# celo-org/celo-bls-snark-rs

Measured on AMD Instinct MI355X. Metric: BLS12-377 G1 MSM scalar-muls/sec, higher is better.
Workload: dtype u32 limbs (28-bit radix, 64-bit column accumulators); 1 GPU; BLS12-377 G1 Pippenger MSM, 2^20 random bases/scalars per GPU, inputs resident in HBM; bases_per_gpu=1048576, window_bits=16, windows=16, buckets=524288

## Files before the change

celo-bls-snark-rs_amd/csrc/host_ifma.cpp:

```cpp
#include <immintrin.h>
#include <cstdint>
#include <cstring>
#include "fp_consts.h"

namespace {

typedef unsigned __int128 u128;
constexpr uint64_t M52 = (uint64_t(1) << 52) - 1;

template <int NL> struct V { __m512i l[NL]; };

template <int N> static bool geq(const uint64_t* a, const uint64_t* b) {
  for (int i = N - 1; i >= 0; i--) if (a[i] != b[i]) return a[i] > b[i];
  return true;
}
template <int N> static void sub_in_place(uint64_t* a, const uint64_t* b) {
  u128 br = 0;
  for (int i = 0; i < N; i++) { u128 d = (u128)a[i] - b[i] - (uint64_t)br; a[i] = (uint64_t)d; br = (d >> 64) & 1; }
}
template <int N> static void dbl_mod(uint64_t* x, const uint64_t* p) {
  uint64_t c = 0;
  for (int i = 0; i < N; i++) { uint64_t n = (x[i] << 1) | c; c = x[i] >> 63; x[i] = n; }
  if (geq<N>(x, p)) sub_in_place<N>(x, p);
}
// ... 120 lines not shown
    return m;
  }

  static inline bool dbl(Vn& a) {
    const Vn U = add(a, a);
    if (maybe_zero(a) & 2u) return false;
    const Vn A1 = pick(U, a, IDX(1, 8 + 0));
    const Vn T1 = mul(A1, A1);
    const Vn XX2 = add(T1, T1), M3 = add(XX2, T1);
    const Vn A2 = pick(U, pick(a, M3, IDX(0, 8 + 1)), IDX(1, 8 + 0, 8 + 1));
    const Vn B2 = pick(T1, M3, IDX(0, 0, 8 + 1));
    const Vn T2 = mul(A2, B2);
    const Vn S2 = add(T2, T2);
    const Vn X3 = sub<1>(pick(T2, T2, IDX(2)), pick(S2, S2, IDX(1)));
    const Vn SmX = sub<2>(pick(T2, T2, IDX(1)), X3);
    const Vn A3 = pick(pick(M3, T2, IDX(1, 8 + 0)), T1, IDX(0, 1, 8 + 0, 1));
    const Vn B3 = pick(SmX, a, IDX(0, 8 + 1, 8 + 2, 8 + 3));
    const Vn T3 = mul(A3, B3);
    const Vn Y3 = sub<0>(T3, pick(T3, T3, IDX(1)));
    a = pick(pick(X3, Y3, IDX(0, 8 + 0)), T3, IDX(0, 1, 8 + 2, 8 + 3));
    return true;
  }
  static inline bool add_pt(Vn& a, const Vn& b, int bo) {
    const Vn A1 = pick(a, b, IDX(0, 8 + bo + 0, 1, 8 + bo + 1, 2, 3));
    const Vn B1 = pick(a, b, IDX(8 + bo + 2, 2, 8 + bo + 3, 3, 8 + bo + 2, 8 + bo + 3));
    const Vn T1 = mul(A1, B1);
    const Vn D = sub<0>(pick(T1, T1, IDX(1, 3)), pick(T1, T1, IDX(0, 2)));
    if (maybe_zero(D) & 1u) return false;
    const Vn T2 = mul(D, D);
    const Vn A3 = pick(D, T1, IDX(0, 8 + 0, 8 + 4));
    const Vn B3 = pick(T2, T2, IDX(0, 0, 0));
    const Vn T3 = mul(A3, B3);
    const Vn Q2 = add(T3, T3);
    const Vn s = add(T3, pick(Q2, Q2, IDX(1)));
    const Vn X3 = sub<2>(pick(T2, T2, IDX(1)), s);
    const Vn QmX = sub<3>(pick(T3, T3, IDX(1)), X3);
    const Vn A4 = pick(D, T1, IDX(1, 8 + 2, 8 + 5));
    const Vn B4 = pick(QmX, T3, IDX(0, 8 + 0, 8 + 0));
    const Vn T4 = mul(A4, B4);
    const Vn Y3 = sub<0>(T4, pick(T4, T4, IDX(1)));
    a = pick(pick(X3, Y3, IDX(0, 8 + 0)), pick(T3, T4, IDX(2, 8 + 2)), IDX(0, 1, 8 + 0, 8 + 1));
    return true;
  }

  static int horner(const uint64_t* pts, size_t stride, const int32_t* order, int steps, uint64_t* out, int* out_inf) {
    const Consts& c = C();
    const Vn cin = bcast(c.c_in), cout = bcast(c.c_out);
    Vn acc;
    for (int j = 0; j < NL; j++) acc.l[j] = _mm512_setzero_si512();
    bool inf = true;
    alignas(64) uint64_t lanes[NL][8];
    for (int k = 0; k < steps; k++) {
      const bool nodbl = order[k] >= 0 && (order[k] & 0x40000000);
      if (!inf && !nodbl && !dbl(acc)) return 1;
      if (order[k] < 0) continue;
      const uint64_t* q = pts + (size_t)(order[k] & 0x3FFFFFFF) * stride;
      uint64_t zz = 0;
      for (int i = 0; i < N; i++) zz |= q[2 * N + i];
      if (zz == 0) continue;
      for (int e = 0; e < 4; e++) {
        uint64_t l[NL];
        to52<N, NL>(q + e * N, l);
        for (int j = 0; j < NL; j++) lanes[j][e] = l[j];
      }
      Vn b;
      for (int j = 0; j < NL; j++) b.l[j] = _mm512_load_si512((const void*)lanes[j]);
      b = mul(b, cin);
      if (inf) { acc = b; inf = false; continue; }
      if (!add_pt(acc, b, 0)) return 1;
    }
    *out_inf = inf ? 1 : 0;
    if (inf) { memset(out, 0, 4 * N * 8); return 0; }
    Vn r = mul(acc, cout);
    for (int j = 0; j < NL; j++) _mm512_store_si512((void*)lanes[j], r.l[j]);
    for (int e = 0; e < 4; e++) {
      uint64_t l[NL], w[N];
      for (int j = 0; j < NL; j++) l[j] = lanes[j][e];
      from52<N, NL>(l, w);
      if (geq<N>(w, P::P64)) sub_in_place<N>(w, P::P64);
      memcpy(out + e * N, w, 8 * N);
    }
    return 0;
  }
};

}

extern "C" int celo_ifma_horner_377(const uint64_t* pts, size_t stride, const int32_t* order, int steps, uint64_t* out, int* inf) {
  return Ifma<celo::P377, 8>::horner(pts, stride, order, steps, out, inf);
}
extern "C" int celo_ifma_horner_761(const uint64_t* pts, size_t stride, const int32_t* order, int steps, uint64_t* out, int* inf) {
  return Ifma<celo::P761, 15>::horner(pts, stride, order, steps, out, inf);
}
```

celo-bls-snark-rs_amd/csrc/msm_engine.h:

```cpp
#pragma once

namespace celo {

extern "C" int celo_ifma_available();
extern "C" int celo_ifma_horner_377(const uint64_t* pts, size_t stride, const int32_t* order, int steps, uint64_t* out, int* inf);
extern "C" int celo_ifma_horner_761(const uint64_t* pts, size_t stride, const int32_t* order, int steps, uint64_t* out, int* inf);
typedef int (*ifma_horner_fn)(const uint64_t*, size_t, const int32_t*, int, uint64_t*, int*);
template <class F> struct IfmaHorner { static constexpr ifma_horner_fn fn = nullptr; };
template <> struct IfmaHorner<Fp<P377>> { static constexpr ifma_horner_fn fn = &celo_ifma_horner_377; };
template <> struct IfmaHorner<Fp<P761>> { static constexpr ifma_horner_fn fn = &celo_ifma_horner_761; };

struct MsmTimings {
  float convert = 0, sort = 0, accumulate = 0, reduce = 0, total = 0;
};

}
#include "msm_ba.h"
namespace celo {
template <> struct BaCfg<G_761> { static constexpr bool enabled = true; };

struct MsmTuning {
  bool narrow_windows, use_glv, use_gls, gls_force, lane_bitsum, host_threads, seg_occupancy, side_convert, side_convert_all, fx_compact;
  uint32_t seg_min, seg_min_shard, bitsum_lanes_max_shard;
  int seg_halves;
  uint32_t bitsum_lanes_max;
  int ba_levels, ba_occ; uint32_t ba_rounds;
  int batched_affine;
  uint32_t host_chunks;
  uint32_t host_head_split, host_tail_split;
  static const MsmTuning& get() {
    static const MsmTuning t = [] {
      MsmTuning v;
      v.use_glv = true;
      v.use_gls = true;
      v.host_chunks = getenv("CELO_HOST_CHUNKS") ? (uint32_t)atoi(getenv("CELO_HOST_CHUNKS")) : 0xFFFFFFFFu;
      v.host_head_split = 0xFFFFFFFFu;
      v.host_tail_split = 0xFFFFFFFFu;
      v.batched_affine = getenv("CELO_BA") ? atoi(getenv("CELO_BA")) : 0;
      v.narrow_windows = true;
      v.gls_force = false;
      v.lane_bitsum = true;
      v.fx_compact = true;
      v.host_threads = true;
      v.seg_halves = 0;
      v.seg_min = 32u;
      v.seg_min_shard = 16u;
      v.seg_occupancy = true;
      v.side_convert = false;
      v.side_convert_all = false;
      v.ba_levels = 3; v.ba_occ = 2; v.ba_rounds = 2u;
      v.bitsum_lanes_max_shard = 21 * 1024;
      v.bitsum_lanes_max = 21 * 1024;
      return v;
    }();
    return t;
  }
};

template <class G> class MsmEngine {
 public:
  typedef typename G::F F;
  typedef PointIO<F> IO;
  static constexpr int SW = G::SCALAR_WORDS;

  ~MsmEngine() { release(); }
  void release() {
    if (arena) { (void)hipFree(arena); arena = nullptr; arena_bytes = 0; }
    if (fxs) { (void)hipFree(fxs); fxs = nullptr; fxs_bytes = 0; }
    for (void* p : {(void*)d_in_bases, (void*)d_in_scalars, (void*)d_in_inf})
      if (p) (void)hipFree(p);
    d_in_bases = nullptr; d_in_scalars = nullptr; d_in_inf = nullptr; cap_in = 0;
    if (h_out) { (void)hipHostFree(h_out); h_out = nullptr; }
    if (d_side_out) { (void)hipFree(d_side_out); d_side_out = nullptr; side_out_bytes = 0; }
    if (d_fx_scalars) { (void)hipFree(d_fx_scalars); d_fx_scalars = nullptr; cap_fx = 0; }
    for (int i = 0; i < 6; i++) if (ev[i]) { (void)hipEventDestroy(ev[i]); ev[i] = nullptr; }
    for (int i = 0; i < 2; i++) if (ev_side[i]) { (void)hipEventDestroy(ev_side[i]); ev_side[i] = nullptr; }
    for (hipEvent_t e : ev_copy) if (e) (void)hipEventDestroy(e);
    ev_copy.clear();
  }
  static int window_bits(size_t n) {
    if (G::SCALAR_BITS > 256) {
      if (n < 512) return 9;
      return n < (size_t(1) << 19) ? 13 : 16;
    }
    if (n < (size_t(1) << 15)) return 11;
    return n < (size_t(1) << 19) ? 15 : 16;
  }
  int force_c = 0;
  hipStream_t own_stream() { return stream_.get(); }
  bool narrow_windows = MsmTuning::get().narrow_windows;
  bool narrow_top(int c) const { return narrow_windows && c == 16; }
  bool big_subgroup_points = false;
  bool ark_zero_identity = false;
// ... 264 lines not shown
      const uint32_t E32 = (uint32_t)fx->E();
      hipLaunchKernelGGL((k_fixed_place<G>), dim3((E32 + 1023) / 1024 < 4096 ? (E32 + 1023) / 1024 : 4096), dim3(1024), 0, stream, d_fx_v8, d_fx_dg, d_fx_cnt + 128, d_digits_all,
                         d_remap, E32, n, fx->NV);
    } else if (fx) hipLaunchKernelGGL((k_fixed_digits<SW, G::SCALAR_BITS>), dim3((fx->n + 255) / 256), dim3(256), 0, stream, d_scalars, fx->tinf, d_digits_all, fx->n, (uint32_t)n_,
                               fx->cf, fx->W, fx->NV, fx->M);
    else if (glv) { if (launch_digits<4, GlvExpand<G>::BITS>(c, (const uint32_t*)(A + o_sc2), nullptr, d_digits_all, n, stream)) return 3; }
    else if (launch_digits<SW, G::SCALAR_BITS>(c, d_scalars, d_inf, d_digits_all, n, stream)) return 3;
    HIP_TRY(hipMemsetAsync(d_counts, 0, o_zero_end - o_counts, stream), 1);
    sort_windows(0, (uint32_t)nw, stream);
    hipLaunchKernelGGL((k_size_hist<G>), dim3(slots / 256 < 512 ? (slots + 255) / 256 : 512), dim3(256), 0, stream, d_plen, d_bins, slots);
    hipLaunchKernelGGL((k_size_scan<G>), dim3(1), dim3(1024), 0, stream, d_bins, d_nwork);
    hipLaunchKernelGGL((k_size_scatter<G>), dim3((slots + 4095) / 4096), dim3(1024), 0, stream, d_plen, d_bins, d_order, slots);
    if (side) HIP_TRY(hipStreamWaitEvent(stream, ev_side[1], 0), 1);
    HIP_TRY(hipEventRecord(ev[2], stream), 1);
    if constexpr (BaCfg<G>::enabled) if (use_ba) {
      uint32_t* d_ba_pts = (uint32_t*)(A + o_ba_pts);
      const int levels = MsmTuning::get().ba_levels;
      if (ba_occ == 2)
        hipLaunchKernelGGL((k_ba_levels<G, 2>), dim3(ba_lanes / 256), dim3(256), 0, stream, d_bases, d_sorted, d_pstart, d_plen, d_order, d_nwork, d_ba_pts,
                           (uint32_t*)(A + o_ba_pref), ba_lanes, levels, ba_pref_slots);
      else
        hipLaunchKernelGGL((k_ba_levels<G, 1>), dim3(ba_lanes / 256), dim3(256), 0, stream, d_bases, d_sorted, d_pstart, d_plen, d_order, d_nwork, d_ba_pts,
                           (uint32_t*)(A + o_ba_pref), ba_lanes, levels, ba_pref_slots);
      hipLaunchKernelGGL((k_accumulate_ba<G>), dim3((slots + 255) / 256), dim3(256), 0, stream, d_ba_pts, d_pstart, d_plen, d_order, d_nwork, d_partials, levels);
    }
    if (!use_ba) launch_accumulate<G>(slots, stream, d_bases, d_sorted, d_pstart, d_plen, d_order, d_nwork, d_partials);
    }
    HIP_TRY(hipEventRecord(ev[3], stream), 1);
    const uint32_t mid_blocks = win_cnt ? (total + 20) / 21 < 16384 ? (total + 20) / 21 : 16384 : 1024;
    const uint32_t cfirst = hin ? 1u : 0u;
    if (lane_bitsum) hipLaunchKernelGGL((k_combine_mid_lanes<G>), dim3(mid_blocks), dim3(64), 0, stream, d_mid, d_nmid, d_counts, d_pfirst, d_partials, d_piecesof, SEG, cfirst);
    else hipLaunchKernelGGL((k_combine_mid<G>), dim3(256), dim3(128), 0, stream, d_mid, d_nmid, d_counts, d_pfirst, d_partials, d_piecesof, SEG, cfirst);
    hipLaunchKernelGGL((k_combine_big<G>), dim3(256), dim3(256), 0, stream, d_big, d_nbig, d_counts, d_pfirst, d_partials, d_piecesof, SEG, cfirst);
    const uint32_t* d_leaf = d_partials;
    const uint32_t* d_leaf_counts = d_counts;
    if (hin) {
      hipLaunchKernelGGL((k_merge_carried<G>), dim3((total + 127) / 128), dim3(128), 0, stream, d_counts, d_pfirst, d_partials, d_carrier, total, K, SEG);
      d_leaf = d_carrier; d_leaf_counts = nullptr;
    }
    {
      struct Arr { uint32_t at, per_window; bool born; int level; };
      uint32_t half_at[2] = {res_pts, res_pts + half_pts};
      Arr tree = {0, B, true, LB};
      std::vector<Arr> lists;
      for (int t = 1; t <= LB; t++) {
        BitsumJobs jobs;
        jobs.njobs = 0;
        uint32_t cursor = half_at[t & 1], total_out = 0;
        auto push = [&](uint32_t src, uint32_t outs_per_window, uint32_t mode, int result_slot) -> uint32_t {
          const uint32_t outs = outs_per_window * (uint32_t)nw;
          uint32_t dst;
          if (result_slot >= 0) dst = (uint32_t)result_slot * (uint32_t)nw;
          else { dst = cursor; cursor += outs; }
          const int j = (int)jobs.njobs++;
          total_out += outs;
          jobs.end[j] = total_out; jobs.src[j] = src; jobs.dst[j] = dst; jobs.mode[j] = mode;
          return dst;
        };
        std::vector<Arr> next_lists;
        if (tree.level >= 2) {
          const uint32_t outs = tree.per_window / 4;
          const uint32_t dst = push(tree.at, outs, tree.level == LB ? 3u : 1u, outs == 1 ? tree.level : -1);
          if (outs > 1) next_lists.push_back({dst, outs, false, tree.level});
        } else {
          push(tree.at, 1, 4u, 1);
        }
        for (const Arr& L : lists) {
          const uint32_t outs = L.per_window / 2;
          const uint32_t dst = push(L.at, outs, 0u, outs == 1 ? L.level : -1);
          if (outs > 1) next_lists.push_back({dst, outs, false, L.level});
        }
        {
          const uint32_t outs = tree.per_window / 2;
          const uint32_t dst = push(tree.at, outs, tree.level == LB ? 2u : 0u, outs == 1 ? 0 : -1);
          tree = {dst, outs, true, tree.level - 1};
        }
        lists.swap(next_lists);
        if (lane_bitsum && total_out <= (win_cnt ? MsmTuning::get().bitsum_lanes_max_shard : BITSUM_LANES_MAX))
          hipLaunchKernelGGL((k_bitsum_lanes<G>), dim3((total_out + 20) / 21), dim3(64), 0, stream, d_leaf, d_leaf_counts, d_pfirst, d_piecesof, SEG, d_work, jobs);
        else
          hipLaunchKernelGGL((k_bitsum<G>), dim3((total_out + 127) / 128), dim3(128), 0, stream, d_leaf, d_leaf_counts, d_pfirst, d_piecesof, SEG,
                             d_work, jobs);
      }
      hipLaunchKernelGGL((k_results_to_ark<G>), dim3((4 * res_pts + 63) / 64), dim3(64), 0, stream, d_work, res_pts);
    }
    HIP_TRY(hipEventRecord(ev[4], stream), 1);
    HIP_TRY(hipMemcpyAsync(h_out, d_work, (size_t)res_pts * IO::XYZZ_WORDS * 4, hipMemcpyDeviceToHost, stream), 1);
    HIP_TRY(hipEventRecord(ev[5], stream), 1);
    HIP_TRY(hipStreamSynchronize(stream), 1);
    HIP_TRY(hipGetLastError(), 1);
    (void)hipEventElapsedTime(&tm.convert, ev[0], ev[1]);
    (void)hipEventElapsedTime(&tm.sort, ev[1], ev[2]);
    (void)hipEventElapsedTime(&tm.accumulate, ev[2], ev[3]);
    (void)hipEventElapsedTime(&tm.reduce, ev[3], ev[4]);
    (void)hipEventElapsedTime(&tm.total, ev[0], ev[5]);
    last_c = c; last_nw = nw; last_buckets = total; last_glv = glv;
    typedef typename HostField<F>::type HF;
    const uint64_t* h64 = reinterpret_cast<const uint64_t*>(h_out);
    constexpr size_t PT64 = (size_t)IO::XYZZ_WORDS / 2;
    horner_steps.clear();
    const int kn = pl.kn;
    (void)sbits;
    if (fx) {
      int top = LB - 1;
      while (((uint64_t)(nw - 1) * fx->M) >> (top + 1)) top++;
      for (int t = top; t >= 0; t--) {
        horner_steps.push_back(-1);
        for (int v = 0; v < nw; v++) if ((((uint64_t)v * fx->M) >> t) & 1) horner_steps.push_back(v | HORNER_NODBL);
        if (t <= LB - 1) for (int v = 0; v < nw; v++) horner_steps.push_back(((LB - t) * nw + v) | HORNER_NODBL);
      }
      for (int v = 0; v < nw; v++) horner_steps.push_back(v | HORNER_NODBL);
    } else
    for (int w = nw - 1; w >= 0; w--) {
      horner_steps.push_back(-1);
      for (int l = (w0 + w >= nw_all - kn ? 2 : 1); l <= LB; l++) horner_steps.push_back(l * nw + w);
      horner_steps.push_back(w | HORNER_NODBL);
    }
    auto run_list = [&](const int32_t* steps, int count) {
      if (IfmaHorner<F>::fn && celo_ifma_available()) {
        uint64_t r[4 * IO::ARK64];
        int inf = 0;
        if (IfmaHorner<F>::fn(h64, PT64, steps, count, r, &inf) == 0) return inf ? HXyzz<HF>::identity() : HXyzz<HF>::load(r, IO::ARK64);
      }
      return host64_horner<HF>(h64, PT64, IO::ARK64, steps, count);
    };
    constexpr int HT = (sizeof(HF) > 6 * 8) ? HOST_HORNER_THREADS : 1;
    HXyzz<HF> total_pt;
    if (HT > 1 && host_threads && (fx ? horner_steps.size() >= 64 : nw >= 2 * HT)) {
      int start[HT + 1], dbls[HT];
      if (fx) {
        int adds_total = 0;
        for (int k = 0; k < (int)horner_steps.size(); k++) adds_total += horner_steps[k] >= 0 ? 1 : 0;
        int g = 0, adds = 0;
        start[0] = 0;
        for (int k = 0; k < (int)horner_steps.size(); k++) {
          if (horner_steps[k] < 0 && g + 1 < HT && k > start[g] && adds * HT >= (g + 1) * adds_total) start[++g] = k;
          adds += horner_steps[k] >= 0 ? 1 : 0;
        }
        while (g + 1 < HT) start[++g] = (int)horner_steps.size();
        start[HT] = (int)horner_steps.size();
        for (int j = 0; j < HT; j++) {
          dbls[j] = 0;
          for (int k = start[j]; k < start[j + 1]; k++) if (horner_steps[k] < 0 || !(horner_steps[k] & HORNER_NODBL)) dbls[j]++;
        }
      } else {
        int wdone = 0, g = 0;
        start[0] = 0;
        for (int k = 0; k < (int)horner_steps.size(); k++) {
          if (horner_steps[k] >= 0 && (horner_steps[k] & HORNER_NODBL)) {
            wdone++;
            if (wdone == (g + 1) * nw / HT && g + 1 < HT) start[++g] = k + 1;
          }
        }
        start[HT] = (int)horner_steps.size();
        for (int j = 0; j < HT; j++) {
          dbls[j] = 0;
          for (int k = start[j]; k < start[j + 1]; k++) if (horner_steps[k] < 0 || !(horner_steps[k] & HORNER_NODBL)) dbls[j]++;
        }
      }
      HXyzz<HF> part[HT];
      std::thread th[HT - 1];
      bool started[HT - 1];
      for (int j = 1; j < HT; j++) {
        started[j - 1] = true;
        try { th[j - 1] = std::thread([&, j] { part[j] = run_list(horner_steps.data() + start[j], start[j + 1] - start[j]); }); }
        catch (const std::system_error&) { started[j - 1] = false; }
      }
      part[0] = run_list(horner_steps.data() + start[0], start[1] - start[0]);
      for (int j = 1; j < HT; j++) {
        if (started[j - 1]) th[j - 1].join();
        else part[j] = run_list(horner_steps.data() + start[j], start[j + 1] - start[j]);
      }
      total_pt = part[0];
      for (int j = 1; j < HT; j++) {
        for (int d = 0; d < dbls[j]; d++) total_pt = hxyzz_dbl(total_pt);
        hxyzz_add(total_pt, part[j]);
      }
    } else {
      total_pt = run_list(horner_steps.data(), (int)horner_steps.size());
    }
    if (out_xyzz) {
      if (total_pt.is_identity()) memset(out_xyzz, 0, 4 * IO::ARK64 * 8);
      else { total_pt.X.store(out_xyzz); total_pt.Y.store(out_xyzz + IO::ARK64); total_pt.ZZ.store(out_xyzz + 2 * IO::ARK64); total_pt.ZZZ.store(out_xyzz + 3 * IO::ARK64); }
    }
    if (out_jac) write_host_jacobian(total_pt, out_jac);
    return 0;
  }
  typedef typename HostField<F>::type HostF;
  static void write_host_jacobian(const HXyzz<HostF>& pt, uint64_t* out_jac) {
    if (pt.is_identity()) { write_identity(out_jac); return; }
    (pt.X * pt.ZZ).store(out_jac);
    (pt.Y * pt.ZZZ).store(out_jac + IO::ARK64);
    pt.ZZ.store(out_jac + 2 * IO::ARK64);
  }

  int run_host(const uint64_t* bases, const uint8_t* inf, const uint64_t* scalars, size_t n, uint64_t* out_jac, hipStream_t stream) {
    return run_host_windows(bases, inf, scalars, n, 0, 0, out_jac, nullptr, stream);
  }
  int run_host_windows(const uint64_t* bases, const uint8_t* inf, const uint64_t* scalars, size_t n, int win_lo, int win_cnt, uint64_t* out_jac,
                       uint64_t* out_xyzz, hipStream_t stream) {
    if (n == 0) return run_device_windows(nullptr, nullptr, nullptr, 0, win_lo, win_cnt, out_jac, out_xyzz, stream);
    const int ovr = host_chunks_override().load();
    const bool fq2_group = sizeof(F) > 14 * sizeof(uint32_t) && G::SCALAR_BITS <= 256;
    uint32_t by_size = (uint32_t)(n >> (fq2_group ? 19 : 18));
    const uint32_t lo_k = G::SCALAR_BITS > 256 ? 8u : 4u, hi_k = fq2_group ? 8u : 16u;
    by_size = by_size < lo_k ? lo_k : by_size > hi_k ? hi_k : by_size;
    uint32_t chunks = ovr >= 0 ? (uint32_t)(ovr & 0xFF) : MsmTuning::get().host_chunks != 0xFFFFFFFFu ? MsmTuning::get().host_chunks : by_size;
    uint32_t head_split = ovr >= 0 && ((ovr >> 8) & 15) ? (uint32_t)((ovr >> 8) & 15) - 1u : MsmTuning::get().host_head_split != 0xFFFFFFFFu ? MsmTuning::get().host_head_split : HOST_HEAD_SPLIT_DEFAULT;
    uint32_t tail_split = ovr >= 0 && ((ovr >> 12) & 15) ? (uint32_t)((ovr >> 12) & 15) - 1u : MsmTuning::get().host_tail_split != 0xFFFFFFFFu ? MsmTuning::get().host_tail_split : HOST_TAIL_SPLIT_DEFAULT;
    if (chunks > 64) chunks = 64;
    const size_t min_chunk_log = ovr >= 0 ? 16 : 17;
    if (chunks > (n >> min_chunk_log)) chunks = (uint32_t)(n >> min_chunk_log);
    const bool glv_plan = plan(n).glv;
    const bool glv_off = glv_plan && !ark_zero_identity && !win_cnt && n >= (size_t(1) << 19);
    if (!(ovr >= 0 && ((ovr >> 8) & 15)) && MsmTuning::get().host_head_split == 0xFFFFFFFFu && chunks && n / chunks < (size_t(1) << 18)) head_split = 0;
    bool pipelined = chunks >= (ovr >= 0 ? 1u : 2u) && !win_cnt && (!glv_plan || glv_off) && n < (size_t(1) << 30) && (!ark_zero_identity || ovr >= 0 || n >= (size_t(1) << 21));
    size_t need = n;
    if (pipelined) {
      uint32_t cm, clen[HOST_CHUNKS_MAX];
      need = (size_t)host_chunk_plan(n, chunks, head_split, tail_split, cm, clen) * cm;
      uint64_t nw_run;
      { struct GlvOff { bool& f; bool was; GlvOff(bool& x, bool off) : f(x), was(x) { if (off) f = false; } ~GlvOff() { f = was; } } g(use_glv, glv_plan);
        nw_run = (uint64_t)plan(n).nw; }
      if ((uint64_t)need * nw_run >= (uint64_t(1) << 32)) { pipelined = false; need = n; }
    }
    const size_t n_real = n;
    n = need;
    if (n > cap_in) {
      if (d_in_bases) (void)hipFree(d_in_bases);
      if (d_in_scalars) (void)hipFree(d_in_scalars);
      if (d_in_inf) (void)hipFree(d_in_inf);
      d_in_bases = nullptr; d_in_scalars = nullptr; d_in_inf = nullptr; cap_in = 0;
      HIP_TRY(hipMalloc(&d_in_bases, n * 2 * IO::ARK64 * 8), 1);
      HIP_TRY(hipMalloc(&d_in_scalars, n * SW * 4), 1);
      HIP_TRY(hipMalloc(&d_in_inf, n), 1);
      cap_in = n;
    }
    n = n_real;
    if (pipelined) {
      const HostIn hin = {bases, inf, scalars, chunks, head_split, tail_split, ark_zero_identity};
      struct GlvOff { bool& f; bool was; GlvOff(bool& x, bool off) : f(x), was(x) { if (off) f = false; } ~GlvOff() { f = was; } } glv_guard(use_glv, glv_plan);
      return run_device_windows(d_in_bases, inf || ark_zero_identity ? d_in_inf : nullptr, (const uint32_t*)d_in_scalars, n, 0, 0, out_jac, out_xyzz, stream, nullptr, &hin);
    }
    HIP_TRY(hipMemcpyAsync(d_in_bases, bases, n * 2 * IO::ARK64 * 8, hipMemcpyHostToDevice, stream), 1);
    HIP_TRY(hipMemcpyAsync(d_in_scalars, scalars, n * SW * 4, hipMemcpyHostToDevice, stream), 1);
    if (inf) HIP_TRY(hipMemcpyAsync(d_in_inf, inf, n, hipMemcpyHostToDevice, stream), 1);
    if (ark_zero_identity) {
      ArkCoord<IO::ARK64> one;
      F::one().to_ark(one.v);
      hipLaunchKernelGGL((k_flag_ark_zero<G>), dim3((unsigned)((n + 255) / 256)), dim3(256), 0, stream, d_in_bases, inf ? d_in_inf : nullptr, d_in_inf, n, one);
      return run_device_windows(d_in_bases, d_in_inf, (const uint32_t*)d_in_scalars, n, win_lo, win_cnt, out_jac, out_xyzz, stream);
    }
    return run_device_windows(d_in_bases, inf ? d_in_inf : nullptr, (const uint32_t*)d_in_scalars, n, win_lo, win_cnt, out_jac, out_xyzz, stream);
  }

  int run_fixed(const FixedTable& T, const void* scalars, size_t n_sc, int resident, uint64_t* out_jac, hipStream_t stream) {
    if (n_sc > T.n) n_sc = T.n;
    if (n_sc == 0) { write_identity(out_jac); return 0; }
    const uint32_t* d_sc = (const uint32_t*)scalars;
    if (!resident) {
      if (n_sc > cap_fx) {
        if (d_fx_scalars) (void)hipFree(d_fx_scalars);
        d_fx_scalars = nullptr; cap_fx = 0;
        HIP_TRY(hipMalloc(&d_fx_scalars, n_sc * SW * 4), 1);
        cap_fx = n_sc;
      }
      HIP_TRY(hipMemcpyAsync(d_fx_scalars, scalars, n_sc * SW * 4, hipMemcpyHostToDevice, stream), 1);
      d_sc = (const uint32_t*)d_fx_scalars;
// ... 182 lines not shown
    HIP_TRY(hipMemsetAsync(d_bins, 0, (size_t)SIZE_BINS * 4 + 256, stream), 1);
    if (nd > 1) {
      uint32_t* d_sc2 = (uint32_t*)(A + o[9]);
      uint8_t* d_inf2 = (uint8_t*)(A + o[10]);
      uint32_t* d_off2 = (uint32_t*)(A + o[11]);
      gls_off.resize(m + 1);
      for (size_t p = 0; p <= m; p++) gls_off[p] = (uint32_t)nd * offsets[p];
      HIP_TRY(hipMemcpyAsync(d_off2, gls_off.data(), (m + 1) * 4, hipMemcpyHostToDevice, stream), 1);
      GlsExpand<G>::launch(d_in_b, inf ? d_in_i : nullptr, d_in_s, d_off, (uint32_t)m, max_n, nd, batch_bits, d_bases, d_sc2, inf ? d_inf2 : nullptr, stream);
      HIP_TRY(hipEventRecord(ev[1], stream), 1);
      if (launch_batch_sort<4>(c, eff_max_n, d_sc2, inf ? d_inf2 : nullptr, d_off2, d_sorted, d_pstart, d_plen, (uint32_t)m, nw, stream)) return 3;
    } else {
      hipLaunchKernelGGL((k_convert_bases<G>), dim3((total_pts + 255) / 256), dim3(256), 0, stream, d_in_b, d_bases, (size_t)total_pts);
      HIP_TRY(hipEventRecord(ev[1], stream), 1);
      if (launch_batch_sort<SW>(c, max_n, d_in_s, inf ? d_in_i : nullptr, d_off, d_sorted, d_pstart, d_plen, (uint32_t)m, nw, stream)) return 3;
    }
    last_gls_digits = nd;
    const uint32_t slots = (uint32_t)nbuckets;
    hipLaunchKernelGGL((k_size_hist<G>), dim3(slots / 256 < 2048 ? (slots + 255) / 256 : 2048), dim3(256), 0, stream, d_plen, d_bins, slots);
    hipLaunchKernelGGL((k_size_scan<G>), dim3(1), dim3(1024), 0, stream, d_bins, d_nwork);
    hipLaunchKernelGGL((k_size_scatter<G>), dim3((slots + 4095) / 4096), dim3(1024), 0, stream, d_plen, d_bins, d_order, slots);
    HIP_TRY(hipEventRecord(ev[2], stream), 1);
    launch_accumulate<G>(slots, stream, d_bases, d_sorted, d_pstart, d_plen, d_order, d_nwork, d_partials);
    HIP_TRY(hipEventRecord(ev[3], stream), 1);
    hipLaunchKernelGGL((k_batch_reduce<G>), dim3(((uint32_t)nvw + 127) / 128), dim3(128), 0, stream, d_partials, d_plen, d_wsum, B, (uint32_t)nvw);
    if (lane_horner) BatchHornerLanes<G>::launch(d_wsum, d_out, (uint32_t)nw, (uint32_t)c, (uint32_t)m, stream);
    else hipLaunchKernelGGL((k_batch_horner<G>), dim3(((uint32_t)m + 127) / 128), dim3(128), 0, stream, d_wsum, d_out, (uint32_t)nw, (uint32_t)c, (uint32_t)m);
    HIP_TRY(hipEventRecord(ev[4], stream), 1);
    if (out) HIP_TRY(hipMemcpyAsync(out, d_out, m * 3 * IO::ARK64 * 8, hipMemcpyDeviceToHost, stream), 1);
    HIP_TRY(hipEventRecord(ev[5], stream), 1);
    last_c = c; last_nw = nw; last_buckets = (uint32_t)nbuckets;
    if (d_out_ret) *d_out_ret = d_out;
    if (!out) { HIP_TRY(hipGetLastError(), 1); return 0; }
    HIP_TRY(hipStreamSynchronize(stream), 1);
    HIP_TRY(hipGetLastError(), 1);
    collect_batch_timings();
    return 0;
  }
  void collect_batch_timings() {
    if (side_path) { tm = tm_batch; return; }
    (void)hipEventElapsedTime(&tm_batch.convert, ev[0], ev[1]);
    (void)hipEventElapsedTime(&tm_batch.sort, ev[1], ev[2]);
    (void)hipEventElapsedTime(&tm_batch.accumulate, ev[2], ev[3]);
    (void)hipEventElapsedTime(&tm_batch.reduce, ev[3], ev[4]);
    (void)hipEventElapsedTime(&tm_batch.total, ev[0], ev[5]);
    tm = tm_batch;
  }

  MsmTimings tm;
  int last_c = 0, last_nw = 0;
  uint32_t last_buckets = 0;

  static void write_identity(uint64_t* out) {
    Xyzz<F> id = Xyzz<F>::identity();
    write_jacobian(id, out);
  }
  static void write_jacobian(const Xyzz<F>& p, uint64_t* out) {
    if (p.is_identity() || p.ZZ.is_zero_mod_p()) {
      F::zero().to_ark(out);
      F::one().to_ark(out + IO::ARK64);
      F::zero().to_ark(out + 2 * IO::ARK64);
      return;
    }
    F::mul(p.X, p.ZZ).to_ark(out);
    F::mul(p.Y, p.ZZZ).to_ark(out + IO::ARK64);
    p.ZZ.to_ark(out + 2 * IO::ARK64);
  }

 private:
  char* arena = nullptr;
  size_t arena_bytes = 0;
  uint64_t* d_in_bases = nullptr;
  uint64_t* d_in_scalars = nullptr;
  uint8_t* d_in_inf = nullptr;
  uint32_t* h_out = nullptr;
  uint64_t* d_fx_scalars = nullptr;
  size_t cap_fx = 0;
  uint8_t* fxs = nullptr;
  size_t fxs_bytes = 0;
  uint64_t* d_side_out = nullptr;
  size_t side_out_bytes = 0;
  bool side_path = false;
  static constexpr size_t H_OUT_POINTS = 17 * 64;
  OwnedStream stream_;
  OwnedStream side_stream_;
  OwnedStream sort_stream_;
  hipEvent_t ev_side[2] = {nullptr, nullptr};
  std::vector<hipEvent_t> ev_copy;
  std::vector<int32_t> horner_steps;
  std::vector<uint32_t> gls_off;
  hipEvent_t ev[6] = {nullptr, nullptr, nullptr, nullptr, nullptr, nullptr};
  size_t cap_in = 0;

  int ensure(size_t bytes) {
    if (!ev[0]) {
      for (int i = 0; i < 6; i++) HIP_TRY(hipEventCreate(&ev[i]), 1);
      for (int i = 0; i < 2; i++) HIP_TRY(hipEventCreateWithFlags(&ev_side[i], hipEventDisableTiming), 1);
    }
    if (!h_out) {
      HIP_TRY(hipHostMalloc(&h_out, H_OUT_POINTS * IO::XYZZ_WORDS * 4), 1);
    }
    if (bytes > arena_bytes) {
      if (arena) (void)hipFree(arena);
      arena = nullptr; arena_bytes = 0;
      HIP_TRY(hipMalloc(&arena, bytes), 1);
      arena_bytes = bytes;
    }
    return 0;
  }

  template <int SWX, int CB, int PT> int launch_batch_sort_cp(const uint32_t* sc, const uint8_t* inf, const uint32_t* off, uint32_t* sorted,
                                                     uint32_t* pstart, uint32_t* plen, uint32_t m, int nw, hipStream_t st) {
    hipLaunchKernelGGL((k_batch_sort<SWX, CB, PT>), dim3(m), dim3(256), 0, st, sc, inf, off, sorted, pstart, plen, nw);
    return 0;
  }
  template <int SWX, int CB> int launch_batch_sort_c(uint32_t max_n, const uint32_t* sc, const uint8_t* inf, const uint32_t* off, uint32_t* sorted,
                                            uint32_t* pstart, uint32_t* plen, uint32_t m, int nw, hipStream_t st) {
    if (max_n <= 256) return launch_batch_sort_cp<SWX, CB, 1>(sc, inf, off, sorted, pstart, plen, m, nw, st);
    if (max_n <= 512) return launch_batch_sort_cp<SWX, CB, 2>(sc, inf, off, sorted, pstart, plen, m, nw, st);
    return launch_batch_sort_cp<SWX, CB, 4>(sc, inf, off, sorted, pstart, plen, m, nw, st);
  }
  template <int SWX> int launch_batch_sort(int c, uint32_t max_n, const uint32_t* sc, const uint8_t* inf, const uint32_t* off, uint32_t* sorted,
                        uint32_t* pstart, uint32_t* plen, uint32_t m, int nw, hipStream_t st) {
    switch (c) {
      case 3: return launch_batch_sort_c<SWX, 3>(max_n, sc, inf, off, sorted, pstart, plen, m, nw, st);
      case 4: return launch_batch_sort_c<SWX, 4>(max_n, sc, inf, off, sorted, pstart, plen, m, nw, st);
      case 5: return launch_batch_sort_c<SWX, 5>(max_n, sc, inf, off, sorted, pstart, plen, m, nw, st);
      case 6: return launch_batch_sort_c<SWX, 6>(max_n, sc, inf, off, sorted, pstart, plen, m, nw, st);
      case 7: return launch_batch_sort_c<SWX, 7>(max_n, sc, inf, off, sorted, pstart, plen, m, nw, st);
      default: return 1;
    }
  }
  template <int SWX, int BITS, int CB> int launch_digits_c(const uint32_t* sc, const uint8_t* inf, uint16_t* digits, uint32_t n, hipStream_t st, uint32_t m, uint32_t npad, uint32_t ibase) {
    constexpr int NW = (BITS + CB) / CB;
    constexpr int KN = NW * CB - (BITS + 1);
    if constexpr (KN > 0 && KN < NW) {
      if (narrow_top(CB)) { hipLaunchKernelGGL((k_digits<SWX, CB, NW, KN, BITS>), dim3((npad - ibase + 255) / 256), dim3(256), 0, st, sc, inf, digits, n, m, npad, ibase); return 0; }
    }
    hipLaunchKernelGGL((k_digits<SWX, CB, NW, 0, BITS>), dim3((npad - ibase + 255) / 256), dim3(256), 0, st, sc, inf, digits, n, m, npad, ibase);
    return 0;
  }
  template <int SWX, int BITS> int launch_digits(int c, const uint32_t* sc, const uint8_t* inf, uint16_t* digits, uint32_t n, hipStream_t st, uint32_t m = 0, uint32_t npad = 0, uint32_t ibase = 0) {
    if (!m) { m = n; npad = n; }
    switch (c) {
      case 4: return launch_digits_c<SWX, BITS, 4>(sc, inf, digits, n, st, m, npad, ibase);
      case 5: return launch_digits_c<SWX, BITS, 5>(sc, inf, digits, n, st, m, npad, ibase);
      case 6: return launch_digits_c<SWX, BITS, 6>(sc, inf, digits, n, st, m, npad, ibase);
      case 7: return launch_digits_c<SWX, BITS, 7>(sc, inf, digits, n, st, m, npad, ibase);
      case 8: return launch_digits_c<SWX, BITS, 8>(sc, inf, digits, n, st, m, npad, ibase);
      case 9: return launch_digits_c<SWX, BITS, 9>(sc, inf, digits, n, st, m, npad, ibase);
      case 10: return launch_digits_c<SWX, BITS, 10>(sc, inf, digits, n, st, m, npad, ibase);
      case 11: return launch_digits_c<SWX, BITS, 11>(sc, inf, digits, n, st, m, npad, ibase);
      case 12: return launch_digits_c<SWX, BITS, 12>(sc, inf, digits, n, st, m, npad, ibase);
      case 13: return launch_digits_c<SWX, BITS, 13>(sc, inf, digits, n, st, m, npad, ibase);
      case 14: return launch_digits_c<SWX, BITS, 14>(sc, inf, digits, n, st, m, npad, ibase);
      case 15: return launch_digits_c<SWX, BITS, 15>(sc, inf, digits, n, st, m, npad, ibase);
      case 16: return launch_digits_c<SWX, BITS, 16>(sc, inf, digits, n, st, m, npad, ibase);
      default: return 1;
    }
  }
};


}
```

celo-bls-snark-rs_amd/csrc/msm_reduce.h:

```cpp
#pragma once

namespace celo {

template <class G>
__global__ void __launch_bounds__(128) k_combine_mid(const uint32_t* __restrict__ mid, const uint32_t* __restrict__ nmid,
                                                     const uint32_t* __restrict__ counts, const uint32_t* __restrict__ pfirst,
                                                     uint32_t* __restrict__ partials, uint32_t* __restrict__ pieces_of, uint32_t SEG, uint32_t first = 0) {
  typedef typename G::F F;
  typedef PointIO<F> IO;
  for (uint32_t q = blockIdx.x * blockDim.x + threadIdx.x; q < *nmid; q += gridDim.x * blockDim.x) {
    uint32_t t = mid[q];
    uint32_t pc = (counts[t] + SEG - 1) / SEG - first, pf = pfirst[t] + first;
    Xyzz<F> acc = IO::load_xyzz(partials + (size_t)pf * IO::XYZZ_WORDS);
    for (uint32_t k = 1; k < pc; k++) {
      Xyzz<F> v = IO::load_xyzz(partials + (size_t)(pf + k) * IO::XYZZ_WORDS);
      xyzz_add_fn(acc, v);
    }
    IO::store_xyzz(partials + (size_t)pf * IO::XYZZ_WORDS, acc);
    pieces_of[t] = 1;
  }
}
template <class G>
__global__ void __launch_bounds__(64) k_combine_mid_lanes(const uint32_t* __restrict__ mid, const uint32_t* __restrict__ nmid,
                                                          const uint32_t* __restrict__ counts, const uint32_t* __restrict__ pfirst,
// ... 57 lines not shown
  typedef typename G::F F;
  typedef PointIO<F> IO;
  if (!counts) return IO::load_xyzz(partials + (size_t)t * IO::XYZZ_WORDS);
  uint32_t c = counts[t];
  if (c == 0) return Xyzz<F>::identity();
  (void)pieces_of; (void)SEG;
  return IO::load_xyzz(partials + (size_t)pfirst[t] * IO::XYZZ_WORDS);
}

struct BitsumJobs {
  static constexpr int MAXJ = 20;
  uint32_t njobs;
  uint32_t end[MAXJ];
  uint32_t src[MAXJ];
  uint32_t dst[MAXJ];
  uint32_t mode[MAXJ];
};
template <class G>
__global__ void __launch_bounds__(128) k_bitsum(const uint32_t* __restrict__ partials, const uint32_t* __restrict__ counts,
                                                const uint32_t* __restrict__ pfirst, const uint32_t* __restrict__ pieces_of, uint32_t SEG,
                                                uint32_t* __restrict__ work, BitsumJobs jobs) {
  typedef typename G::F F;
  typedef PointIO<F> IO;
  const uint32_t t = blockIdx.x * blockDim.x + threadIdx.x;
  if (t >= jobs.end[jobs.njobs - 1]) return;
  uint32_t j = 0;
  while (t >= jobs.end[j]) j++;
  const uint32_t i = t - (j ? jobs.end[j - 1] : 0u);
  const uint32_t mode = jobs.mode[j];
  Xyzz<F> a, b;
  if (mode == 2) {
    a = load_bucket<G>(partials, counts, pfirst, pieces_of, 2 * i, SEG);
    b = load_bucket<G>(partials, counts, pfirst, pieces_of, 2 * i + 1, SEG);
  } else if (mode == 3) {
    a = load_bucket<G>(partials, counts, pfirst, pieces_of, 4 * i + 1, SEG);
    b = load_bucket<G>(partials, counts, pfirst, pieces_of, 4 * i + 3, SEG);
  } else {
    const uint32_t* in = work + (size_t)jobs.src[j] * IO::XYZZ_WORDS;
    const size_t ia = mode == 0 ? 2 * (size_t)i : mode == 1 ? 4 * (size_t)i + 1 : 2 * (size_t)i + 1;
    a = IO::load_xyzz(in + ia * IO::XYZZ_WORDS);
    if (mode != 4) b = IO::load_xyzz(in + (ia + (mode == 0 ? 1 : 2)) * IO::XYZZ_WORDS);
  }
  if (mode != 4) xyzz_add(a, b);
  IO::store_xyzz(work + ((size_t)jobs.dst[j] + i) * IO::XYZZ_WORDS, a);
}
template <class G>
__global__ void __launch_bounds__(64) k_bitsum_lanes(const uint32_t* __restrict__ partials, const uint32_t* __restrict__ counts,
                                                     const uint32_t* __restrict__ pfirst, const uint32_t* __restrict__ pieces_of, uint32_t SEG,
                                                     uint32_t* __restrict__ work, BitsumJobs jobs) {
  typedef typename G::F F;
  typedef PointIO<F> IO;
  typedef QTriT<FieldBase<F>> QB;
  typedef LanePoint<QB> LP;
  const int g = QB::group();
  const uint32_t t = blockIdx.x * 21u + (uint32_t)g;
  if (g >= 21 || t >= jobs.end[jobs.njobs - 1]) return;
  uint32_t j = 0;
  while (t >= jobs.end[j]) j++;
  const uint32_t i = t - (j ? jobs.end[j - 1] : 0u);
  const uint32_t mode = jobs.mode[j];
  Xyzz<F> a, b = Xyzz<F>::identity();
  if (mode == 2) {
    a = load_bucket<G>(partials, counts, pfirst, pieces_of, 2 * i, SEG);
    b = load_bucket<G>(partials, counts, pfirst, pieces_of, 2 * i + 1, SEG);
  } else if (mode == 3) {
    a = load_bucket<G>(partials, counts, pfirst, pieces_of, 4 * i + 1, SEG);
    b = load_bucket<G>(partials, counts, pfirst, pieces_of, 4 * i + 3, SEG);
  } else {
    const uint32_t* in = work + (size_t)jobs.src[j] * IO::XYZZ_WORDS;
    const size_t ia = mode == 0 ? 2 * (size_t)i : mode == 1 ? 4 * (size_t)i + 1 : 2 * (size_t)i + 1;
    a = IO::load_xyzz(in + ia * IO::XYZZ_WORDS);
    if (mode != 4) b = IO::load_xyzz(in + (ia + (mode == 0 ? 1 : 2)) * IO::XYZZ_WORDS);
  }
  typename LP::Pt acc = {{a.X, a.Y, a.ZZ, a.ZZZ}, a.is_identity()};
  if (mode != 4) {
    const typename LP::P pb = {b.X, b.Y, b.ZZ, b.ZZZ};
    LP::add(acc, pb, b.is_identity());
  }
  if (QB::lane() != 0) return;
  const Xyzz<F> r = acc.inf ? Xyzz<F>::identity() : Xyzz<F>{acc.p.X, acc.p.Y, acc.p.ZZ, acc.p.ZZZ};
  IO::store_xyzz(work + ((size_t)jobs.dst[j] + i) * IO::XYZZ_WORDS, r);
}
template <class G>
__global__ void __launch_bounds__(64) k_results_to_ark(uint32_t* __restrict__ work, uint32_t res_pts) {
  typedef typename G::F F;
  typedef PointIO<F> IO;
  const uint32_t t = blockIdx.x * blockDim.x + threadIdx.x, pt = t >> 2, q = t & 3;
  const bool live = pt < res_pts;
  uint64_t out[IO::ARK64];
  if (live) F::load(work + (size_t)pt * IO::XYZZ_WORDS + q * IO::FW).to_ark(out);
  __syncthreads();
  if (live) {
    uint64_t* o = reinterpret_cast<uint64_t*>(work + (size_t)pt * IO::XYZZ_WORDS) + q * IO::ARK64;
#pragma unroll
    for (int i = 0; i < IO::ARK64; i++) o[i] = out[i];
  }
}

}
```

Baseline: 318.4 million scalar-muls/s.

## Write results to mapped host memory, spin on seq flag, add 8-lane IFMA Horner

The final GPU kernel now writes converted results straight into mapped, coherent pinned host memory and raises a sequence flag. The host spins on that flag instead of doing a memcpy plus stream synchronize, which removes copy and sync latency from the critical path. Event timing reads move after the host work. Separately, the host-side Horner combine of window results now runs 8 window groups in parallel across AVX-512 IFMA lanes, then joins the partial results with a second short Horner pass instead of using threads. The risks are busy-wait CPU use, reliance on the blocks_done counter being reset between calls, and extra multiplies from the 8-lane formulas.

```diff
diff --git a/celo-bls-snark-rs_amd/csrc/host_ifma.cpp b/celo-bls-snark-rs_amd/csrc/host_ifma.cpp
--- a/celo-bls-snark-rs_amd/csrc/host_ifma.cpp
+++ b/celo-bls-snark-rs_amd/csrc/host_ifma.cpp
@@ -226,6 +226,108 @@
     }
     return 0;
   }
+
+  struct Pt8 { Vn X, Y, ZZ, ZZZ; };
+  __attribute__((noinline)) static Vn mulv(const Vn& a, const Vn& b) { return mul(a, b); }
+  static inline void keep(Vn& a, const Vn& r, unsigned live) {
+    for (int j = 0; j < NL; j++) a.l[j] = _mm512_mask_mov_epi64(a.l[j], (__mmask8)live, r.l[j]);
+  }
+  static bool dbl8(Pt8& a, unsigned live) {
+    if (maybe_zero(a.Y) & live) return false;
+    const Vn U = add(a.Y, a.Y);
+    const Vn Vv = mulv(U, U), XX = mulv(a.X, a.X);
+    const Vn M = add(add(XX, XX), XX);
+    const Vn W = mulv(U, Vv), S = mulv(a.X, Vv), M2 = mulv(M, M);
+    const Vn X3 = sub<1>(M2, add(S, S));
+    const Vn SmX = sub<2>(S, X3);
+    const Vn Y3 = sub<0>(mulv(M, SmX), mulv(W, a.Y));
+    keep(a.ZZ, mulv(Vv, a.ZZ), live);
+    keep(a.ZZZ, mulv(W, a.ZZZ), live);
+    keep(a.X, X3, live);
+    keep(a.Y, Y3, live);
+    return true;
+  }
+  static bool add8(Pt8& a, const Pt8& b, unsigned live) {
+    const Vn U1 = mulv(a.X, b.ZZ), U2 = mulv(b.X, a.ZZ), S1 = mulv(a.Y, b.ZZZ), S2 = mulv(b.Y, a.ZZZ);
+    const Vn Pd = sub<0>(U2, U1), R = sub<0>(S2, S1);
+    if (maybe_zero(Pd) & live) return false;
+    const Vn ZZp = mulv(a.ZZ, b.ZZ), ZZZp = mulv(a.ZZZ, b.ZZZ);
+    const Vn PP = mulv(Pd, Pd), R2 = mulv(R, R);
+    const Vn PPP = mulv(Pd, PP), Q = mulv(U1, PP);
+    const Vn X3 = sub<2>(R2, add(PPP, add(Q, Q)));
+    const Vn QmX = sub<3>(Q, X3);
+    const Vn Y3 = sub<0>(mulv(R, QmX), mulv(S1, PPP));
+    keep(a.ZZ, mulv(ZZp, PP), live);
+    keep(a.ZZZ, mulv(ZZZp, PPP), live);
+    keep(a.X, X3, live);
+    keep(a.Y, Y3, live);
+    return true;
+  }
+  static int horner8(const uint64_t* pts, size_t stride, const int32_t* order, const int32_t* start, int groups, uint64_t* out, int* out_inf) {
+    if (groups < 1 || groups > 8) return 1;
+    const Consts& c = C();
+    const Vn cin = bcast(c.c_in), cout = bcast(c.c_out);
+    Pt8 acc;
+    for (int j = 0; j < NL; j++) acc.X.l[j] = acc.Y.l[j] = acc.ZZ.l[j] = acc.ZZZ.l[j] = _mm512_setzero_si512();
+    unsigned inf = 0xFFu;
+    int rounds = 0;
+    for (int g = 0; g < groups; g++) {
+      if (start[g + 1] < start[g]) return 1;
+      if (start[g + 1] - start[g] > rounds) rounds = start[g + 1] - start[g];
+    }
+    alignas(64) uint64_t st[4][NL][8];
+    memset(st, 0, sizeof(st));
+    for (int r = 0; r < rounds; r++) {
+      unsigned md = 0, ma = 0;
+      for (int g = 0; g < groups; g++) {
+        if (start[g] + r >= start[g + 1]) continue;
+        const int32_t s = order[start[g] + r];
+        const bool nodbl = s >= 0 && (s & 0x40000000);
+        if (!nodbl && !((inf >> g) & 1u)) md |= 1u << g;
+        if (s < 0) continue;
+        const uint64_t* q = pts + (size_t)(s & 0x3FFFFFFF) * stride;
+        uint64_t zz = 0;
+        for (int i = 0; i < N; i++) zz |= q[2 * N + i];
+        if (zz == 0) continue;
+        ma |= 1u << g;
+        for (int e = 0; e < 4; e++) {
+          uint64_t l[NL];
+          to52<N, NL>(q + e * N, l);
+          for (int j = 0; j < NL; j++) st[e][j][g] = l[j];
+        }
+      }
+      if (md && !dbl8(acc, md)) return 1;
+      if (!ma) continue;
+      Pt8 b;
+      Vn* bv[4] = {&b.X, &b.Y, &b.ZZ, &b.ZZZ};
+      for (int e = 0; e < 4; e++) {
+        Vn raw;
+        for (int j = 0; j < NL; j++) raw.l[j] = _mm512_load_si512((const void*)st[e][j]);
+        *bv[e] = mulv(raw, cin);
+      }
+      const unsigned first = ma & inf, live = ma & ~inf;
+      if (live && !add8(acc, b, live)) return 1;
+      if (first) {
+        keep(acc.X, b.X, first); keep(acc.Y, b.Y, first); keep(acc.ZZ, b.ZZ, first); keep(acc.ZZZ, b.ZZZ, first);
+        inf &= ~first;
+      }
+    }
+    const Vn* av[4] = {&acc.X, &acc.Y, &acc.ZZ, &acc.ZZZ};
+    for (int e = 0; e < 4; e++) {
+      const Vn r = mulv(*av[e], cout);
+      for (int j = 0; j < NL; j++) _mm512_store_si512((void*)st[0][j], r.l[j]);
+      for (int g = 0; g < groups; g++) {
+        uint64_t l[NL], w[N];
+        for (int j = 0; j < NL; j++) l[j] = st[0][j][g];
+        from52<N, NL>(l, w);
+        if (geq<N>(w, P::P64)) sub_in_place<N>(w, P::P64);
+        if ((inf >> g) & 1u) memset(w, 0, 8 * N);
+        memcpy(out + ((size_t)g * 4 + e) * N, w, 8 * N);
+      }
+    }
+    for (int g = 0; g < groups; g++) out_inf[g] = (int)((inf >> g) & 1u);
+    return 0;
+  }
 };
 
 }
@@ -233,6 +335,9 @@
 extern "C" int celo_ifma_horner_377(const uint64_t* pts, size_t stride, const int32_t* order, int steps, uint64_t* out, int* inf) {
   return Ifma<celo::P377, 8>::horner(pts, stride, order, steps, out, inf);
 }
+extern "C" int celo_ifma_horner8_377(const uint64_t* pts, size_t stride, const int32_t* order, const int32_t* start, int groups, uint64_t* out, int* inf) {
+  return Ifma<celo::P377, 8>::horner8(pts, stride, order, start, groups, out, inf);
+}
 extern "C" int celo_ifma_horner_761(const uint64_t* pts, size_t stride, const int32_t* order, int steps, uint64_t* out, int* inf) {
   return Ifma<celo::P761, 15>::horner(pts, stride, order, steps, out, inf);
 }
diff --git a/celo-bls-snark-rs_amd/csrc/msm_engine.h b/celo-bls-snark-rs_amd/csrc/msm_engine.h
--- a/celo-bls-snark-rs_amd/csrc/msm_engine.h
+++ b/celo-bls-snark-rs_amd/csrc/msm_engine.h
@@ -1,4 +1,5 @@
 #pragma once
+#include <chrono>
 
 namespace celo {
 
@@ -9,6 +10,10 @@
 template <class F> struct IfmaHorner { static constexpr ifma_horner_fn fn = nullptr; };
 template <> struct IfmaHorner<Fp<P377>> { static constexpr ifma_horner_fn fn = &celo_ifma_horner_377; };
 template <> struct IfmaHorner<Fp<P761>> { static constexpr ifma_horner_fn fn = &celo_ifma_horner_761; };
+extern "C" int celo_ifma_horner8_377(const uint64_t* pts, size_t stride, const int32_t* order, const int32_t* start, int groups, uint64_t* out, int* inf);
+typedef int (*ifma_horner8_fn)(const uint64_t*, size_t, const int32_t*, const int32_t*, int, uint64_t*, int*);
+template <class F> struct IfmaHorner8 { static constexpr ifma_horner8_fn fn = nullptr; };
+template <> struct IfmaHorner8<Fp<P377>> { static constexpr ifma_horner8_fn fn = &celo_ifma_horner8_377; };
 
 struct MsmTimings {
   float convert = 0, sort = 0, accumulate = 0, reduce = 0, total = 0;
@@ -439,18 +444,22 @@
           hipLaunchKernelGGL((k_bitsum<G>), dim3((total_out + 127) / 128), dim3(128), 0, stream, d_leaf, d_leaf_counts, d_pfirst, d_piecesof, SEG,
                              d_work, jobs);
       }
-      hipLaunchKernelGGL((k_results_to_ark<G>), dim3((4 * res_pts + 63) / 64), dim3(64), 0, stream, d_work, res_pts);
-    }
+    }
+    const uint32_t seq = ++result_seq ? result_seq : ++result_seq;
+    hipLaunchKernelGGL((k_results_to_host<G>), dim3((4 * res_pts + 63) / 64), dim3(64), 0, stream, d_work, res_pts, reinterpret_cast<uint64_t*>(h_out),
+                       d_bins + SIZE_BINS + 3, h_seq(), seq);
     HIP_TRY(hipEventRecord(ev[4], stream), 1);
-    HIP_TRY(hipMemcpyAsync(h_out, d_work, (size_t)res_pts * IO::XYZZ_WORDS * 4, hipMemcpyDeviceToHost, stream), 1);
     HIP_TRY(hipEventRecord(ev[5], stream), 1);
-    HIP_TRY(hipStreamSynchronize(stream), 1);
     HIP_TRY(hipGetLastError(), 1);
-    (void)hipEventElapsedTime(&tm.convert, ev[0], ev[1]);
-    (void)hipEventElapsedTime(&tm.sort, ev[1], ev[2]);
-    (void)hipEventElapsedTime(&tm.accumulate, ev[2], ev[3]);
-    (void)hipEventElapsedTime(&tm.reduce, ev[3], ev[4]);
-    (void)hipEventElapsedTime(&tm.total, ev[0], ev[5]);
+    {
+      const auto t_end = std::chrono::steady_clock::now() + std::chrono::milliseconds(RESULT_SPIN_MS);
+      bool seen = false;
+      while (!seen) {
+        for (int k = 0; k < 512 && !seen; k++) seen = __atomic_load_n(h_seq(), __ATOMIC_ACQUIRE) == seq;
+        if (!seen && std::chrono::steady_clock::now() >= t_end) break;
+      }
+      if (!seen) HIP_TRY(hipStreamSynchronize(stream), 1);
+    }
     last_c = c; last_nw = nw; last_buckets = total; last_glv = glv;
     typedef typename HostField<F>::type HF;
     const uint64_t* h64 = reinterpret_cast<const uint64_t*>(h_out);
@@ -482,8 +491,44 @@
       return host64_horner<HF>(h64, PT64, IO::ARK64, steps, count);
     };
     constexpr int HT = (sizeof(HF) > 6 * 8) ? HOST_HORNER_THREADS : 1;
+    auto cut_windows = [&](int groups, int* start, int* dbls) {
+      int wdone = 0, g = 0;
+      start[0] = 0;
+      for (int k = 0; k < (int)horner_steps.size(); k++) {
+        if (horner_steps[k] >= 0 && (horner_steps[k] & HORNER_NODBL)) {
+          wdone++;
+          if (wdone == (g + 1) * nw / groups && g + 1 < groups) start[++g] = k + 1;
+        }
+      }
+      start[groups] = (int)horner_steps.size();
+      for (int j = 0; j < groups; j++) {
+        dbls[j] = 0;
+        for (int k = start[j]; k < start[j + 1]; k++) if (horner_steps[k] < 0 || !(horner_steps[k] & HORNER_NODBL)) dbls[j]++;
+      }
+    };
     HXyzz<HF> total_pt;
-    if (HT > 1 && host_threads && (fx ? horner_steps.size() >= 64 : nw >= 2 * HT)) {
+    bool joined8 = false;
+    if (IfmaHorner8<F>::fn && !fx && nw >= 8 && celo_ifma_available()) {
+      constexpr int H8 = 8;
+      int start[H8 + 1], dbls[H8], inf8[H8];
+      uint64_t r[H8 * 4 * IO::ARK64];
+      cut_windows(H8, start, dbls);
+      if (IfmaHorner8<F>::fn(h64, PT64, horner_steps.data(), start, H8, r, inf8) == 0) {
+        std::vector<int32_t>& js = join_steps;
+        js.clear();
+        for (int j = 0; j < H8; j++) {
+          for (int d = 1; j && d < dbls[j]; d++) js.push_back(-1);
+          js.push_back(j && dbls[j] ? j : j | HORNER_NODBL);
+        }
+        uint64_t t[4 * IO::ARK64];
+        int inf = 0;
+        if (IfmaHorner<F>::fn(r, 4 * IO::ARK64, js.data(), (int)js.size(), t, &inf) == 0) total_pt = inf ? HXyzz<HF>::identity() : HXyzz<HF>::load(t, IO::ARK64);
+        else total_pt = host64_horner<HF>(r, 4 * IO::ARK64, IO::ARK64, js.data(), (int)js.size());
+        joined8 = true;
+      }
+    }
+    if (joined8) {
+    } else if (HT > 1 && host_threads && (fx ? horner_steps.size() >= 64 : nw >= 2 * HT)) {
       int start[HT + 1], dbls[HT];
       if (fx) {
         int adds_total = 0;
@@ -500,21 +545,7 @@
           dbls[j] = 0;
           for (int k = start[j]; k < start[j + 1]; k++) if (horner_steps[k] < 0 || !(horner_steps[k] & HORNER_NODBL)) dbls[j]++;
         }
-      } else {
-        int wdone = 0, g = 0;
-        start[0] = 0;
-        for (int k = 0; k < (int)horner_steps.size(); k++) {
-          if (horner_steps[k] >= 0 && (horner_steps[k] & HORNER_NODBL)) {
-            wdone++;
-            if (wdone == (g + 1) * nw / HT && g + 1 < HT) start[++g] = k + 1;
-          }
-        }
-        start[HT] = (int)horner_steps.size();
-        for (int j = 0; j < HT; j++) {
-          dbls[j] = 0;
-          for (int k = start[j]; k < start[j + 1]; k++) if (horner_steps[k] < 0 || !(horner_steps[k] & HORNER_NODBL)) dbls[j]++;
-        }
-      }
+      } else cut_windows(HT, start, dbls);
       HXyzz<HF> part[HT];
       std::thread th[HT - 1];
       bool started[HT - 1];
@@ -541,6 +572,13 @@
       else { total_pt.X.store(out_xyzz); total_pt.Y.store(out_xyzz + IO::ARK64); total_pt.ZZ.store(out_xyzz + 2 * IO::ARK64); total_pt.ZZZ.store(out_xyzz + 3 * IO::ARK64); }
     }
     if (out_jac) write_host_jacobian(total_pt, out_jac);
+    HIP_TRY(hipEventSynchronize(ev[5]), 1);
+    HIP_TRY(hipGetLastError(), 1);
+    (void)hipEventElapsedTime(&tm.convert, ev[0], ev[1]);
+    (void)hipEventElapsedTime(&tm.sort, ev[1], ev[2]);
+    (void)hipEventElapsedTime(&tm.accumulate, ev[2], ev[3]);
+    (void)hipEventElapsedTime(&tm.reduce, ev[3], ev[4]);
+    (void)hipEventElapsedTime(&tm.total, ev[0], ev[5]);
     return 0;
   }
   typedef typename HostField<F>::type HostF;
@@ -889,12 +927,16 @@
   size_t side_out_bytes = 0;
   bool side_path = false;
   static constexpr size_t H_OUT_POINTS = 17 * 64;
+  uint32_t* h_seq() const { return h_out + H_OUT_POINTS * IO::XYZZ_WORDS; }
+  uint32_t result_seq = 0;
+  static constexpr int RESULT_SPIN_MS = 50;
   OwnedStream stream_;
   OwnedStream side_stream_;
   OwnedStream sort_stream_;
   hipEvent_t ev_side[2] = {nullptr, nullptr};
   std::vector<hipEvent_t> ev_copy;
   std::vector<int32_t> horner_steps;
+  std::vector<int32_t> join_steps;
   std::vector<uint32_t> gls_off;
   hipEvent_t ev[6] = {nullptr, nullptr, nullptr, nullptr, nullptr, nullptr};
   size_t cap_in = 0;
@@ -905,7 +947,9 @@
       for (int i = 0; i < 2; i++) HIP_TRY(hipEventCreateWithFlags(&ev_side[i], hipEventDisableTiming), 1);
     }
     if (!h_out) {
-      HIP_TRY(hipHostMalloc(&h_out, H_OUT_POINTS * IO::XYZZ_WORDS * 4), 1);
+      HIP_TRY(hipHostMalloc(&h_out, H_OUT_POINTS * IO::XYZZ_WORDS * 4 + 64, hipHostMallocMapped | hipHostMallocCoherent), 1);
+      *h_seq() = 0;
+      result_seq = 0;
     }
     if (bytes > arena_bytes) {
       if (arena) (void)hipFree(arena);
diff --git a/celo-bls-snark-rs_amd/csrc/msm_reduce.h b/celo-bls-snark-rs_amd/csrc/msm_reduce.h
--- a/celo-bls-snark-rs_amd/csrc/msm_reduce.h
+++ b/celo-bls-snark-rs_amd/csrc/msm_reduce.h
@@ -163,19 +163,22 @@
   IO::store_xyzz(work + ((size_t)jobs.dst[j] + i) * IO::XYZZ_WORDS, r);
 }
 template <class G>
-__global__ void __launch_bounds__(64) k_results_to_ark(uint32_t* __restrict__ work, uint32_t res_pts) {
+__global__ void __launch_bounds__(64) k_results_to_host(const uint32_t* __restrict__ work, uint32_t res_pts, uint64_t* __restrict__ host_out,
+                                                        uint32_t* __restrict__ blocks_done, uint32_t* host_seq, uint32_t seq) {
   typedef typename G::F F;
   typedef PointIO<F> IO;
   const uint32_t t = blockIdx.x * blockDim.x + threadIdx.x, pt = t >> 2, q = t & 3;
-  const bool live = pt < res_pts;
-  uint64_t out[IO::ARK64];
-  if (live) F::load(work + (size_t)pt * IO::XYZZ_WORDS + q * IO::FW).to_ark(out);
-  __syncthreads();
-  if (live) {
-    uint64_t* o = reinterpret_cast<uint64_t*>(work + (size_t)pt * IO::XYZZ_WORDS) + q * IO::ARK64;
+  if (pt < res_pts) {
+    uint64_t out[IO::ARK64];
+    F::load(work + (size_t)pt * IO::XYZZ_WORDS + q * IO::FW).to_ark(out);
+    uint64_t* o = host_out + (size_t)pt * (IO::XYZZ_WORDS / 2) + q * IO::ARK64;
 #pragma unroll
     for (int i = 0; i < IO::ARK64; i++) o[i] = out[i];
   }
+  __threadfence_system();
+  __syncthreads();
+  if (threadIdx.x == 0 && __hip_atomic_fetch_add(blocks_done, 1u, __ATOMIC_ACQ_REL, __HIP_MEMORY_SCOPE_AGENT) == gridDim.x - 1)
+    __hip_atomic_store(host_seq, seq, __ATOMIC_RELEASE, __HIP_MEMORY_SCOPE_SYSTEM);
 }
 
 }
```

Result: faster. 322.7 million scalar-muls/s, median of 6 (+1.3%).
